# kyutai-labs/moshi

Measured on AMD Instinct MI355X. Metric: 12.5 Hz frames/s end-to-end Mimi+Moshi-7B, higher is better.
Workload: dtype bf16

## Files before the change

moshi_amd/csrc/lm_engine.hip:

```cpp
#include "lm_kernels.h"
#include "mmi_graph.h"

#include <math.h>
#include <stdio.h>
#include <map>

namespace {

struct GemmW {
    u32x4* wp = nullptr;
    int N = 0, K = 0, NT = 0, KSTEPS = 0, gate = 0;
    float* scale = nullptr;
    float* scb = nullptr;
    int wq = 0;
    int ksteps = 0;
    uint8_t* s4 = nullptr;
    float xinv = 1.f;
    size_t bytes = 0;
    int T = 32;
};

struct LayerW {
    GemmW in_proj, out_proj, ffn_in, ffn_out;
    uint16_t *n1 = nullptr, *n2 = nullptr;
// ... 2224 lines not shown
        mx = off[b] > mx ? off[b] : mx;
    }
    hipStream_t s = (hipStream_t)stream;
    MMI_HIP_CHECK(hipStreamSynchronize(s));
    MMI_HIP_CHECK(hipMemcpy(lm->offsets, off.data(), (size_t)G * sizeof(long), hipMemcpyHostToDevice));
    if (lm->offsets_m != lm->offsets) MMI_HIP_CHECK(hipMemcpy(lm->offsets_m, off.data(), (size_t)lm->batch * sizeof(long), hipMemcpyHostToDevice));
    lm->offset_cpu = mx;
    lm->depth_bound = mx;
    return MMI_OK;
}

#define MMI_DBG_HIP(call)                                                                                          \
    do {                                                                                                           \
        hipError_t e_ = (call);                                                                                    \
        if (e_ != hipSuccess) return done(mmi_fail(MMI_ERR_HIP, std::string(#call) + ": " + hipGetErrorString(e_))); \
    } while (0)
#define MMI_DBG_LAUNCHED()                                                                                         \
    do {                                                                                                           \
        hipError_t e_ = hipGetLastError();                                                                         \
        if (e_ != hipSuccess) return done(mmi_fail(MMI_ERR_HIP, std::string("kernel launch failed: ") + hipGetErrorString(e_))); \
    } while (0)

extern "C" int mmi_lm_debug_linear(mmi_lm* lm, const char* weight_name, const char* alpha_name, int32_t path, const void* x_bf16,
                                   int32_t rows, void* out_bf16, int8_t* codes, float* absmax, void* norm_out, mmi_stream stream) {
    MmiDeviceGuard dev_guard_(lm ? lm->device : -1);
    if (!lm || !weight_name || !x_bf16 || !out_bf16) return mmi_fail(MMI_ERR_INVALID, "null argument");
    if (rows <= 0 || rows > lm->max_batch) return mmi_fail(MMI_ERR_SHAPE, "mmi_lm_debug_linear: rows must be 1..max_batch");
    auto it = lm->linear_by_name.find(weight_name);
    if (it == lm->linear_by_name.end()) return mmi_fail(MMI_ERR_MISSING_WEIGHT, std::string("no packed linear named ") + weight_name);
    const GemmW g = it->second;
    const uint16_t* alpha = nullptr;
    const bool normed = path == MMI_DBG_NORM || path == MMI_DBG_NORM_FUSED;
    if (normed) {
        auto ia = alpha_name ? lm->vector_by_name.find(alpha_name) : lm->vector_by_name.end();
        if (ia == lm->vector_by_name.end()) return mmi_fail(MMI_ERR_MISSING_WEIGHT, "mmi_lm_debug_linear: the norm's alpha vector was not found");
        alpha = ia->second;
    }
    const bool a8 = act8_of(lm);
    if ((codes || absmax) && !(a8 && (path == MMI_DBG_PLAIN || path == MMI_DBG_SPLITK || path == MMI_DBG_NORM)))
        return mmi_fail(MMI_ERR_UNSUPPORTED, "mmi_lm_debug_linear: codes / absmax exist on the int8 x int8 paths that materialise the operand (plain, split-K, norm)");
    hipStream_t s = (hipStream_t)stream;
    const int T = g.T, mt = mmi_cdiv(rows, T), KS = mmi_kstep(T);
    if (mt > 2 && (path == MMI_DBG_FUSED || path == MMI_DBG_NORM_FUSED))
        return mmi_fail(MMI_ERR_UNSUPPORTED, "mmi_lm_debug_linear: the fused forms are not selected above 64 rows (k_gemm_rows + a norm launch)");
    const int K = g.K, N = g.N, kin = packed_ksteps_t(lm, T, K), kout = packed_ksteps_t(lm, T, N);
    const int nthK = [&] { int n = mmi_cdiv(K / 8, 64) * 64; return n > 1024 ? 1024 : n; }();
    MmiArena A;
    A.poison = lm->knobs.debug_poison;
    uint16_t *xp = nullptr, *yp = nullptr, *xres = nullptr, *zeros = nullptr, *outp = (uint16_t*)out_bf16;
    uint8_t* xq = nullptr;
    float *sx = nullptr, *partial = nullptr;
    const size_t xelems = (size_t)mt * kin * 512, oelems = (size_t)mt * kout * 512;
    bool ok = true;
    ok &= hipSuccess == A.alloc(&xp, xelems);
    ok &= hipSuccess == A.alloc(&yp, xelems);
    ok &= hipSuccess == A.alloc(&xq, (size_t)mt * (kin / 2 + 1) * 1024);
    ok &= hipSuccess == A.alloc(&sx, (size_t)mt * T);
    ok &= hipSuccess == A.alloc(&xres, oelems);
    ok &= hipSuccess == A.alloc(&zeros, (size_t)N + 8);
    ok &= hipSuccess == A.alloc(&partial, (size_t)4 * rows * N);
    auto done = [&](int rc) { hipStreamSynchronize(s); A.release(); return rc; };
    if (!ok) return done(mmi_fail(MMI_ERR_HIP, "out of device memory (mmi_lm_debug_linear)"));
    MMI_DBG_HIP(hipMemsetAsync(xp, 0, xelems * 2, s));
    MMI_DBG_HIP(hipMemsetAsync(yp, 0, xelems * 2, s));
    MMI_DBG_HIP(hipMemsetAsync(xq, 0, (size_t)mt * (kin / 2 + 1) * 1024, s));
    MMI_DBG_HIP(hipMemsetAsync(sx, 0, (size_t)mt * T * sizeof(float), s));
    MMI_DBG_HIP(hipMemsetAsync(xres, 0, oelems * 2, s));
    MMI_DBG_HIP(hipMemsetAsync(zeros, 0, ((size_t)N + 8) * 2, s));
    MMI_LAUNCH(k_pack_rows, mmi_cdiv(rows * K, 256), 256, 0, s, (const uint16_t*)x_bf16, rows, K, xp, T, kin);
    MMI_DBG_LAUNCHED();
    const uint16_t* operand = xp;
    const bool gated = g.gate != 0;
    GemmArgs a;
    memset(&a, 0, sizeof(a));
    a.out = outp; a.epi = gated ? MMI_EPI_GATE : MMI_EPI_STORE; a.B = rows; a.tok_rows = rows;
    a.out_mode = MMI_OUT_ROWMAJOR; a.out_ld = N; a.out_ksteps = kout;
    int rc = MMI_OK;
    if (path == MMI_DBG_NORM) {
        MMI_LAUNCH(k_resid_rmsnorm, rows, nthK, 0, s, xp, (const float*)nullptr, 0, rows, alpha, yp, K, T, kin, 1e-8f,
                   a8 ? xq : (uint8_t*)nullptr, a8 ? sx : (float*)nullptr, (const float*)nullptr, (const float*)nullptr);
        MMI_DBG_LAUNCHED();
        operand = yp;
        if (norm_out) MMI_LAUNCH(k_unpack_rows, mmi_cdiv(rows * K, 256), 256, 0, s, (const uint16_t*)yp, rows, K, (uint16_t*)norm_out, T, kin);
    } else if (a8 && (path == MMI_DBG_PLAIN || path == MMI_DBG_SPLITK)) {
        MMI_LAUNCH(k_quant_rows_i8, rows, nthK, 0, s, (const uint16_t*)xp, rows, K, T, kin, xq, sx);
        MMI_DBG_LAUNCHED();
    }
    if (path == MMI_DBG_PLAIN || path == MMI_DBG_NORM || path == MMI_DBG_SPLITK) {
        a.xp = reinterpret_cast<const u32x4*>(operand);
        if (a8) { a.xp = reinterpret_cast<const u32x4*>(xq); a.sx = sx; a.wq = 3; }
        Pending pd;
        if (path == MMI_DBG_SPLITK) {
            const GemmPlan p = plan_gemm(lm->knobs, g, true);
            if (gated || p.ksplit <= 1) return done(mmi_fail(MMI_ERR_UNSUPPORTED, "mmi_lm_debug_linear: the engine does not split this GEMM over K"));
            a.epi = MMI_EPI_PARTIAL; a.partial = partial; a.out = nullptr;
            pd.P = p.ksplit;
            if (a8) { pd.sx = sx; pd.scb = g.scb; }
        }
        rc = launch_gemm(lm, s, g, a, false);
        if (rc) return done(rc);
        if (path == MMI_DBG_SPLITK) {
            const int nthN = [&] { int n = mmi_cdiv(N / 8, 64) * 64; return n > 1024 ? 1024 : n; }();
            if (N > 8 * 1024 * MMI_NORM_MAXP) return done(mmi_fail(MMI_ERR_UNSUPPORTED, "row too long for the norm kernel"));
            uint16_t* ytmp = nullptr;
            if (A.alloc(&ytmp, oelems) != hipSuccess) return done(mmi_fail(MMI_ERR_HIP, "out of device memory"));
            MMI_LAUNCH(k_resid_rmsnorm, rows, nthN, 0, s, xres, (const float*)partial, pd.P, rows, (const uint16_t*)zeros, ytmp, N, T, kout, 1e-8f,
                       (uint8_t*)nullptr, (float*)nullptr, pd.sx, pd.scb);
            MMI_LAUNCH(k_unpack_rows, mmi_cdiv(rows * N, 256), 256, 0, s, (const uint16_t*)xres, rows, N, outp, T, kout);
            MMI_DBG_LAUNCHED();
        }
    } else if (path == MMI_DBG_FUSED) {
        const int kmax = q8_fused_kmax(g);
        if (!a8 || !kmax) return done(mmi_fail(MMI_ERR_UNSUPPORTED, "mmi_lm_debug_linear: k_gemm_q8 needs an int8 x int8 model and rows of <= 88 entries"));
        a.xp = reinterpret_cast<const u32x4*>(xp);
        a.wp = g.wp; a.N = g.N; a.KSTEPS = g.KSTEPS; a.NT = g.NT; a.wscale = g.scale; a.wscb = g.scb; a.gate_rows = gated ? g.N : 0;
        a.wq = 3; a.xinv = g.xinv;
        a.osplit = q8_fused_osplit(lm->knobs, g, a.epi, T);
        rc = launch_q8_fused(s, T, mt, kmax, g.NT * a.osplit, !lm->knobs.q8_tiles_serial, a);
        if (rc) return done(rc);
    } else if (path == MMI_DBG_NORM_FUSED) {
        const int wq = (a8 && g.wq == 1) ? 3 : g.wq;
        if (g.KSTEPS > norm_fused_max(wq)) return done(mmi_fail(MMI_ERR_UNSUPPORTED, "mmi_lm_debug_linear: the row is too long for the norm-fused GEMM"));
        a.xp = reinterpret_cast<const u32x4*>(xp);
        a.alpha = alpha; a.D = K; a.eps = 1e-8f;
        a.wp = g.wp; a.N = g.N; a.KSTEPS = g.KSTEPS; a.NT = g.NT; a.wscale = g.scale; a.wscb = g.scb; a.ws4 = g.s4; a.gate_rows = gated ? g.N : 0;
        a.wq = wq; a.xinv = g.xinv; a.osplit = 1;
        rc = launch_norm_fused(s, T, mt, wq, g.NT, !lm->knobs.q8_tiles_serial, a);
        if (rc) return done(rc);
    } else {
        return done(mmi_fail(MMI_ERR_INVALID, "mmi_lm_debug_linear: unknown path"));
    }
    if (codes) MMI_LAUNCH(k_unpack_q8, mmi_cdiv(rows * K, 256), 256, 0, s, (const uint8_t*)xq, rows, K, codes, T, kin);
    if (absmax) MMI_DBG_HIP(hipMemcpyAsync(absmax, sx, (size_t)rows * sizeof(float), hipMemcpyDeviceToDevice, s));
    MMI_DBG_LAUNCHED();
    (void)KS;
    if (hipStreamSynchronize(s) != hipSuccess) { A.release(); return mmi_fail(MMI_ERR_HIP, "mmi_lm_debug_linear: the launches failed"); }
    A.release();
    return MMI_OK;
}

extern "C" int64_t mmi_lm_stat(const mmi_lm* lm, int32_t which) {
    MmiDeviceGuard dev_guard_(lm ? lm->device : -1);
    if (!lm) return -1;
    if (which == 0) return (int64_t)lm->xlds_launches;
    if (which == 1) {
        int64_t m = 0;
        for (int v = 0; v < MmiProgram::NV; ++v)
            if (lm->prog.ready(v, false) || lm->prog.ready(v, true)) m |= 1ll << v;
        return m;
    }
    if (which == 2) return (int64_t)lm->depth_bound;
    if (which == 3) return (int64_t)lm->Td;
    if (which == 4) return (int64_t)lm->rows_launches;
    return -1;
}

extern "C" int mmi_lm_profile_begin(mmi_lm* lm) {
    MmiDeviceGuard dev_guard_(lm ? lm->device : -1);
    if (!lm) return mmi_fail(MMI_ERR_INVALID, "null handle");
    lm->profiling = true;
    lm->ev_used = 0;
    lm->site_ev_used = 0;
    lm->prog.tap = [lm](size_t i, bool begin, hipStream_t s) {
        if (!begin && i + 1 != lm->prog.ops.size()) return;
        if (lm->site_ev_used == lm->site_ev.size()) {
            mmi_lm::SiteEv e{0, nullptr};
            if (hipEventCreate(&e.ev) != hipSuccess) return;
            lm->site_ev.push_back(e);
        }
        lm->site_ev[lm->site_ev_used].op = begin ? i : (size_t)-1;
        hipEventRecord(lm->site_ev[lm->site_ev_used].ev, s);
        lm->site_ev_used += 1;
    };
    return MMI_OK;
}

extern "C" int64_t mmi_lm_profile_sites(mmi_lm* lm, char* buf, int64_t cap) {
    MmiDeviceGuard dev_guard_(lm ? lm->device : -1);
    if (!lm || !lm->profiling) return 0;
    if (lm->prof_stream) hipStreamSynchronize(lm->prof_stream);
    else hipDeviceSynchronize();
    std::vector<std::string> order;
    std::vector<double> tot;
    std::vector<long> cnt, bytes;
    for (size_t k = 0; k + 1 < lm->site_ev_used; ++k) {
        const auto& e = lm->site_ev[k];
        if (e.op == (size_t)-1) continue;
        float ms = 0.f;
        if (hipEventElapsedTime(&ms, e.ev, lm->site_ev[k + 1].ev) != hipSuccess) continue;
        const std::string& site = lm->prog.sites[e.op];
        size_t j = 0;
        while (j < order.size() && order[j] != site) ++j;
        if (j == order.size()) { order.push_back(site); tot.push_back(0.0); cnt.push_back(0); bytes.push_back(0); }
        tot[j] += ms; cnt[j] += 1;
        if (lm->prog.op_bytes[e.op] > bytes[j]) bytes[j] = lm->prog.op_bytes[e.op];
    }
    (void)hipGetLastError();
    std::string all;
    for (size_t j = 0; j < order.size(); ++j)
        all += order[j] + "\t" + std::to_string(cnt[j]) + "\t" + std::to_string(tot[j]) + "\t" + std::to_string(bytes[j]) + "\n";
    const int64_t need = (int64_t)all.size() + 1;
    if (buf && cap > 0) {
        const int64_t n = need <= cap ? need - 1 : cap - 1;
        memcpy(buf, all.data(), (size_t)n);
        buf[n] = 0;
    }
    return need;
}

extern "C" int mmi_lm_profile_end(mmi_lm* lm, double* mean_ms, int64_t* n_launches, int64_t* bytes_per_launch,
                                  const char** kernel_name) {
    MmiDeviceGuard dev_guard_(lm ? lm->device : -1);
    if (!lm) return mmi_fail(MMI_ERR_INVALID, "null handle");
    if (!lm->profiling) return mmi_fail(MMI_ERR_STATE, "profiling was not started");
    lm->profiling = false;
    lm->prog.tap = nullptr;
    if (lm->prof_stream || lm->ev_used) MMI_HIP_CHECK(hipStreamSynchronize(lm->prof_stream));
    double tot = 0.0;
    for (size_t i = 0; i < lm->ev_used; ++i) {
        float ms = 0.f;
        MMI_HIP_CHECK(hipEventElapsedTime(&ms, lm->ev_pool[i].a, lm->ev_pool[i].b));
        tot += ms;
    }
    if (mean_ms) *mean_ms = lm->ev_used ? tot / (double)lm->ev_used : 0.0;
    if (n_launches) *n_launches = (int64_t)lm->ev_used;
    if (bytes_per_launch) {
        const mmi_lm_cfg& c = lm->cfg;
        const int64_t wbytes = lm->q8 == 4 ? (int64_t)2 * c.ffn_hidden * c.dim / 2 + (int64_t)2 * c.ffn_hidden * c.dim / 16
                               : lm->q8 >= 1 ? (int64_t)2 * c.ffn_hidden * c.dim + (int64_t)2 * c.ffn_hidden * 4 : (int64_t)2 * c.ffn_hidden * c.dim * 2;
        *bytes_per_launch = wbytes + (int64_t)lm->batch * c.dim * 2 + (int64_t)lm->batch * c.ffn_hidden * 2;
    }
    if (kernel_name)
        *kernel_name = lm->act8      ? "k_gemm_xp<32, MT, 1, 8, 2, 3> (temporal FFN linear_in, int8 weights x int8 activations on v_mfma_i32_32x32x32_i8 + SiLU gate)"
                       : lm->q8 == 1 ? "k_gemm_xp<32, 1, 1, 8, 2, 1> (temporal FFN linear_in, int8 weights + SiLU gate)"
                       : lm->q8 == 4 ? "k_gemm_xp<32, MT, 1, 8, U, 4> (temporal FFN linear_in, MXFP4 weights widened to bf16 + SiLU gate)"
                       : lm->q8 == 2 ? "k_gemm_xp<32, 1, 1, 8, 2, 2> (temporal FFN linear_in, fp8 weights on the fp8 MFMA + SiLU gate)"
                       : lm->dominant_xlds ? (lm->batch > 32 ? "k_gemm_xlds<2, 32, 3, true, 0> (temporal FFN linear_in + SiLU gate)"
                                                             : "k_gemm_xlds<1, 64, 3, true, 0> (temporal FFN linear_in + SiLU gate)")
                                     : "k_gemm_xp<32, 1, 1, 8, 2> (temporal FFN linear_in + SiLU gate)";
    lm->ev_used = 0;
    return MMI_OK;
}
```

moshi_amd/csrc/lm_kernels.h:

```cpp
#pragma once
#include "mmi_common.h"
#include "mmi_fp4.h"

MMI_HD long mmi_xp_index(int T, int b, int k, int ksteps) {
    const int sh = T == 32 ? 4 : 5;
    const int mt = b / T, bl = b - mt * T;
    const int ks = k >> sh, kq = (k >> 3) & ((1 << (sh - 3)) - 1), e = k & 7;
    return ((((long)mt * ksteps + ks) * 64) + kq * T + bl) * 8 + e;
}
static inline int mmi_kstep(int T) { return T == 32 ? 16 : 32; }

__global__ void k_pack_w_bf16(const uint16_t* __restrict__ W, uint16_t* __restrict__ P, int N, int K, int TN, int NT,
                              int KSTEPS, int gate_hidden) {
    long idx = (long)blockIdx.x * blockDim.x + threadIdx.x;
    long total = (long)NT * KSTEPS * 512;
    if (idx >= total) return;
    int e = (int)(idx & 7);
    int lane = (int)((idx >> 3) & 63);
    long rest = idx >> 9;
    int ks = (int)(rest % KSTEPS);
    int nt = (int)(rest / KSTEPS);
    int i, kq, kstep;
    if (TN == 32) { i = lane & 31; kq = lane >> 5; kstep = 16; } else { i = lane & 15; kq = lane >> 4; kstep = 32; }
    int k = ks * kstep + 8 * kq + e;
// ... 1521 lines not shown
    float max_period;
    unsigned* done;
    int solo_rows;
};

#define MMI_ATTN_CHUNK 256
template <int DH, bool KV8 = false>
__global__ __launch_bounds__(256) void k_lm_attn_split(LmAttnArgs a) {
    constexpr int EPL = KV8 ? 16 : 8;
    constexpr int ES = KV8 ? 1 : 2;
    constexpr int LPR = DH / EPL;
    constexpr int RPW = 64 / LPR;
    constexpr int CH = MMI_ATTN_CHUNK;
    const int bh = blockIdx.x;
    const int b = bh / a.H;
    const int tid = threadIdx.x, wave = tid >> 6, lane = tid & 63;
    const long off = a.offsets[b];
    const long end_new = off + 1;
    const int end_index = (int)(off % a.cap);
    const int L = (int)(end_new < (long)a.cap ? end_new : (long)a.cap);
    MMI_SHARED float sc[CH];
    MMI_SHARED float wred[8];
    MMI_SHARED float ored[4 * DH];
    const int seg = lane % LPR, rsub = lane / LPR;
    float qv[EPL];
#pragma unroll
    for (int v = 0; v < EPL / 8; ++v) {
        u32x4 qq = *reinterpret_cast<const u32x4*>(a.qrot + (long)bh * DH + seg * EPL + v * 8);
#pragma unroll
        for (int q = 0; q < 4; ++q) {
            qv[v * 8 + 2 * q] = mmi_bf16_to_f32((uint16_t)(qq[q] & 0xffffu));
            qv[v * 8 + 2 * q + 1] = mmi_bf16_to_f32((uint16_t)(qq[q] >> 16));
        }
    }
    auto widen = [](const u32x4& r, float* f) {
        if constexpr (KV8) {
#pragma unroll
            for (int q = 0; q < 4; ++q) mmi_fp8x4_to_f32(r[q], f + 4 * q);
        } else {
#pragma unroll
            for (int q = 0; q < 4; ++q) {
                f[2 * q] = mmi_bf16_to_f32((uint16_t)(r[q] & 0xffffu));
                f[2 * q + 1] = mmi_bf16_to_f32((uint16_t)(r[q] >> 16));
            }
        }
    };
    const uint8_t* kbase = reinterpret_cast<const uint8_t*>(a.kc) + (long)bh * a.cap * DH * ES;
    const uint8_t* vbase = reinterpret_cast<const uint8_t*>(a.vc) + (long)bh * a.cap * DH * ES;
    const float scale = 1.0f / sqrtf((float)DH);
    constexpr int PER_WAVE = CH / 4;
    float m_run = -INFINITY, l_run = 0.f;
    float acc[EPL];
#pragma unroll
    for (int e = 0; e < EPL; ++e) acc[e] = 0.f;
    for (int c0 = (int)blockIdx.y * CH; c0 < L; c0 += (int)gridDim.y * CH) {
        constexpr int NIT = PER_WAVE / RPW;
        constexpr int NB = NIT < 8 ? NIT : 8;
#pragma unroll 1
        for (int h0 = 0; h0 < NIT; h0 += NB) {
            u32x4 kk[NB];
#pragma unroll
            for (int i = 0; i < NB; ++i) {
                const int slot = min(c0 + wave * PER_WAVE + (h0 + i) * RPW + rsub, L - 1);
                kk[i] = *reinterpret_cast<const u32x4*>(kbase + ((long)slot * DH + seg * EPL) * ES);
            }
#pragma unroll
            for (int i = 0; i < NB; ++i) {
                const int rl = wave * PER_WAVE + (h0 + i) * RPW + rsub;
                const int slot = c0 + rl;
                bool valid = slot < L;
                if (valid) {
                    int delta = slot - end_index;
                    long pos = delta <= 0 ? off + delta : off + delta - a.cap;
                    long dq = off - pos;
                    valid = pos >= 0 && dq >= 0 && dq < a.context;
                }
                float dot = 0.f;
                float kf[EPL];
                widen(kk[i], kf);
#pragma unroll
                for (int e = 0; e < EPL; ++e) dot += qv[e] * kf[e];
#pragma unroll
                for (int m = LPR / 2; m >= 1; m >>= 1) dot += mmi_shfl_xor(dot, m);
                if (seg == 0) sc[rl] = valid ? dot * scale : -INFINITY;
            }
        }
        __syncthreads();
        const float sv = sc[tid];
        float mx = sv;
#pragma unroll
        for (int m = 32; m >= 1; m >>= 1) mx = fmaxf(mx, mmi_shfl_xor(mx, m));
        if (lane == 0) wred[wave] = mx;
        __syncthreads();
        mx = fmaxf(fmaxf(wred[0], wred[1]), fmaxf(wred[2], wred[3]));
        const float m_new = fmaxf(m_run, mx);
        const float p = (m_new == -INFINITY) ? 0.f : expf(sv - m_new);
        float sum = p;
#pragma unroll
        for (int m = 32; m >= 1; m >>= 1) sum += mmi_shfl_xor(sum, m);
        if (lane == 0) wred[4 + wave] = sum;
        sc[tid] = p;
        __syncthreads();
        sum = (wred[4] + wred[5]) + (wred[6] + wred[7]);
        const float resc = (m_run == -INFINITY) ? 0.f : expf(m_run - m_new);
        l_run = l_run * resc + sum;
        m_run = m_new;
#pragma unroll
        for (int e = 0; e < EPL; ++e) acc[e] *= resc;
#pragma unroll 1
        for (int h0 = 0; h0 < NIT; h0 += NB) {
            u32x4 vv[NB];
#pragma unroll
            for (int i = 0; i < NB; ++i) {
                const int slot = min(c0 + wave * PER_WAVE + (h0 + i) * RPW + rsub, L - 1);
                vv[i] = *reinterpret_cast<const u32x4*>(vbase + ((long)slot * DH + seg * EPL) * ES);
            }
#pragma unroll
            for (int i = 0; i < NB; ++i) {
                const int rl = wave * PER_WAVE + (h0 + i) * RPW + rsub;
                const float pr = (c0 + rl < L) ? sc[rl] : 0.f;
                float vf[EPL];
                widen(vv[i], vf);
#pragma unroll
                for (int e = 0; e < EPL; ++e) acc[e] += pr * vf[e];
            }
        }
        __syncthreads();
    }
#pragma unroll
    for (int e = 0; e < EPL; ++e)
#pragma unroll
        for (int m = 32; m >= LPR; m >>= 1) acc[e] += mmi_shfl_xor(acc[e], m);
    if (rsub == 0) {
#pragma unroll
        for (int e = 0; e < EPL; ++e) ored[wave * DH + seg * EPL + e] = acc[e];
    }
    __syncthreads();
    if (tid < DH) {
        const float o = (ored[tid] + ored[DH + tid]) + (ored[2 * DH + tid] + ored[3 * DH + tid]);
        if (gridDim.y == 1) {
            a.out[mmi_xp_index(a.T, b, (bh % a.H) * DH + tid, a.out_ksteps)] = mmi_f32_to_bf16(o / l_run);
        } else {
            a.opart[((long)bh * gridDim.y + blockIdx.y) * DH + tid] = o;
        }
    }
    if (gridDim.y > 1 && tid == 0) {
        float* mlp = a.ml + ((long)bh * gridDim.y + blockIdx.y) * 2;
        mlp[0] = m_run;
        mlp[1] = l_run;
    }
}

template <int DH, bool KV8 = false>
__global__ __launch_bounds__(256, KV8 ? 2 : 4) void k_lm_attn_wave(LmAttnArgs a) {
    constexpr int EPL = KV8 ? 16 : 8;
    constexpr int ES = KV8 ? 1 : 2;
    constexpr int LPR = DH / EPL;
    constexpr int RPW = 64 / LPR;
    constexpr int NB = 4;
    const int bh = blockIdx.x;
    const int b = bh / a.H;
    const int tid = threadIdx.x, wave = tid >> 6, lane = tid & 63;
    const long off = a.offsets[b];
    const int end_index = (int)(off % a.cap);
    const long end_new = off + 1;
    const int L = (int)(end_new < (long)a.cap ? end_new : (long)a.cap);
    const int seg = lane % LPR, rsub = lane / LPR;
    float qv[EPL];
    u32x4 qp = {0u, 0u, 0u, 0u};
#pragma unroll
    for (int v = 0; v < EPL / 8; ++v) {
        u32x4 qq = *reinterpret_cast<const u32x4*>(a.qrot + (long)bh * DH + seg * EPL + v * 8);
        if (v == 0) qp = qq;
#pragma unroll
        for (int q = 0; q < 4; ++q) {
            qv[v * 8 + 2 * q] = mmi_bf16_to_f32((uint16_t)(qq[q] & 0xffffu));
            qv[v * 8 + 2 * q + 1] = mmi_bf16_to_f32((uint16_t)(qq[q] >> 16));
        }
    }
    auto widen = [](const u32x4& r, float* f) {
        if constexpr (KV8) {
#pragma unroll
            for (int q = 0; q < 4; ++q) mmi_fp8x4_to_f32(r[q], f + 4 * q);
        } else {
#pragma unroll
            for (int q = 0; q < 4; ++q) {
                f[2 * q] = mmi_bf16_to_f32((uint16_t)(r[q] & 0xffffu));
                f[2 * q + 1] = mmi_bf16_to_f32((uint16_t)(r[q] >> 16));
            }
        }
    };
    const uint8_t* kbase = reinterpret_cast<const uint8_t*>(a.kc) + (long)bh * a.cap * DH * ES;
    const uint8_t* vbase = reinterpret_cast<const uint8_t*>(a.vc) + (long)bh * a.cap * DH * ES;
    const unsigned loff = (unsigned)(seg * EPL * ES);
    const float scale = 1.0f / sqrtf((float)DH);
    u32x4 kA[NB], vA[NB], kB[NB], vB[NB];
    const bool early = gridDim.y == 1;
    if (early) {
#pragma unroll
        for (int i = 0; i < NB; ++i) {
            const int slot_ = min((wave + i * 4) * RPW + rsub, a.cap - 1);
            const unsigned o_ = (unsigned)slot_ * (unsigned)(DH * ES) + loff;
            kA[i] = *reinterpret_cast<const u32x4*>(kbase + o_);
            vA[i] = *reinterpret_cast<const u32x4*>(vbase + o_);
        }
    }
    const bool windowed = a.context < a.cap;
    const bool solo = (int)gridDim.y > 1 && L <= a.solo_rows;
    if (solo && blockIdx.y != 0) return;
    const int nsplit = solo ? 1 : (int)gridDim.y;
    const int total = nsplit * 4, wg = (solo ? 0 : (int)blockIdx.y * 4) + wave;
    const int ngroups = (L + RPW - 1) / RPW;
    const int nmine = wg < ngroups ? (ngroups - wg + total - 1) / total : 0;
    const int nrounds = (nmine + NB - 1) / NB;
    float m_run = -INFINITY, l_run = 0.f, acc[EPL];
#pragma unroll
    for (int e = 0; e < EPL; ++e) acc[e] = 0.f;
#define MMI_AW_LOAD(KK, VV, j0)                                                                  \
    _Pragma("unroll") for (int i = 0; i < NB; ++i) {                                            \
        const int slot_ = min((wg + ((j0) + i) * total) * RPW + rsub, L - 1);                   \
        const unsigned o_ = (unsigned)slot_ * (unsigned)(DH * ES) + loff;                       \
        KK[i] = *reinterpret_cast<const u32x4*>(kbase + o_);                                    \
        VV[i] = *reinterpret_cast<const u32x4*>(vbase + o_);                                    \
    }
#define MMI_AW_USE(KK, VV, j0)                                                                   \
    {                                                                                            \
        float s_[NB];                                                                            \
        float mx_ = -INFINITY;                                                                   \
        _Pragma("unroll") for (int i = 0; i < NB; ++i) {                                        \
            const int j_ = (j0) + i;                                                             \
            const int slot_ = (wg + j_ * total) * RPW + rsub;                                    \
            bool valid_ = j_ < nmine && slot_ < L;                                               \
            if (windowed && valid_) {    \
                const int delta_ = slot_ - end_index;                                            \
                const long pos_ = delta_ <= 0 ? off + delta_ : off + delta_ - a.cap;             \
                const long dq_ = off - pos_;                                                     \
                valid_ = pos_ >= 0 && dq_ >= 0 && dq_ < a.context;                               \
            }                                                                                    \
            float dot_ = 0.f;                                                                    \
            if constexpr (KV8) {                                                                 \
                float kf_[EPL];                                                                  \
                widen(KK[i], kf_);                                                               \
                _Pragma("unroll") for (int e = 0; e < EPL; ++e) dot_ = mmi_fma(qv[e], kf_[e], dot_); \
            } else {                     \
                _Pragma("unroll") for (int q = 0; q < 4; ++q) dot_ = mmi_dot2_bf16(KK[i][q], qp[q], dot_); \
            }                                                                                    \
            dot_ = mmi_group_sum<LPR>(dot_);                 \
            s_[i] = valid_ ? dot_ * scale : -INFINITY;                                           \
            mx_ = fmaxf(mx_, s_[i]);                                                             \
        }                                                                                        \
        const float m_new_ = fmaxf(m_run, mx_);                                                  \
        if (m_new_ != -INFINITY) {                                                               \
            const float resc_ = m_run == -INFINITY ? 0.f : expf(m_run - m_new_);                 \
            l_run *= resc_;                                                                      \
            _Pragma("unroll") for (int e = 0; e < EPL; ++e) acc[e] *= resc_;                    \
            _Pragma("unroll") for (int i = 0; i < NB; ++i) {                                    \
                const float p_ = expf(s_[i] - m_new_);         \
                l_run += p_;                                                                     \
                if constexpr (KV8) {                                                             \
                    float vf_[EPL];                                                              \
                    widen(VV[i], vf_);                                                           \
                    _Pragma("unroll") for (int e = 0; e < EPL; ++e) acc[e] = mmi_fma(p_, vf_[e], acc[e]); \
                } else {                 \
                    const f32x2 pp_ = {p_, p_};                                                  \
                    _Pragma("unroll") for (int q = 0; q < 4; ++q) {                             \
                        const f32x2 v2_ = {__builtin_bit_cast(float, VV[i][q] << 16), __builtin_bit_cast(float, VV[i][q] & 0xffff0000u)}; \
                        const f32x2 a2_ = mmi_pk_fma(pp_, v2_, f32x2{acc[2 * q], acc[2 * q + 1]}); \
                        acc[2 * q] = a2_[0];                                                     \
                        acc[2 * q + 1] = a2_[1];                                                 \
                    }                                                                            \
                }                                                                                \
            }                                                                                    \
            m_run = m_new_;                                                                      \
        }                                                                                        \
    }
    if (nrounds > 0) {
        if (!early) { MMI_AW_LOAD(kA, vA, 0) }
        for (int r = 0; r < nrounds; r += 2) {
            MMI_AW_LOAD(kB, vB, (r + 1) * NB)
            MMI_AW_USE(kA, vA, r * NB)
            MMI_AW_LOAD(kA, vA, (r + 2) * NB)
            MMI_AW_USE(kB, vB, (r + 1) * NB)
        }
    }
#undef MMI_AW_LOAD
#undef MMI_AW_USE
#pragma unroll
    for (int mk = LPR; mk < 64; mk <<= 1) {
        const float mo = mmi_shfl_xor(m_run, mk), lo = mmi_shfl_xor(l_run, mk);
        const float mn = fmaxf(m_run, mo);
        const float sa = m_run == -INFINITY ? 0.f : expf(m_run - mn), sb = mo == -INFINITY ? 0.f : expf(mo - mn);
        l_run = l_run * sa + lo * sb;
#pragma unroll
        for (int e = 0; e < EPL; ++e) acc[e] = acc[e] * sa + mmi_shfl_xor(acc[e], mk) * sb;
        m_run = mn;
    }
    MMI_SHARED float wm[4], wl[4];
    MMI_SHARED float wacc[4 * DH];
    if (rsub == 0) {
#pragma unroll
        for (int e = 0; e < EPL; ++e) wacc[wave * DH + seg * EPL + e] = acc[e];
        if (seg == 0) { wm[wave] = m_run; wl[wave] = l_run; }
    }
    __syncthreads();
    if (tid < DH) {
        const float M = fmaxf(fmaxf(wm[0], wm[1]), fmaxf(wm[2], wm[3]));
        float num = 0.f, den = 0.f;
#pragma unroll
        for (int w = 0; w < 4; ++w) {
            const float sw = wm[w] == -INFINITY ? 0.f : expf(wm[w] - M);
            num += sw * wacc[w * DH + tid];
            den += sw * wl[w];
        }
        if (nsplit == 1) {
            a.out[mmi_xp_index(a.T, b, (bh % a.H) * DH + tid, a.out_ksteps)] = mmi_f32_to_bf16(num / den);
        } else {
            a.opart[((long)bh * gridDim.y + blockIdx.y) * DH + tid] = num;
            if (tid == 0) {
                float* mlp = a.ml + ((long)bh * gridDim.y + blockIdx.y) * 2;
                mlp[0] = M;
                mlp[1] = den;
            }
        }
    }
    if (nsplit == 1 || a.done == nullptr) return;
    MMI_SHARED unsigned s_last;
    __syncthreads();
    if (tid == 0) {
        const unsigned seen = mmi_arrive_release(a.done + bh);
        s_last = seen == (unsigned)gridDim.y - 1u ? 1u : 0u;
        if (s_last) {
            mmi_store_relaxed_agent(a.done + bh, 0u);
            mmi_acquire_agent();
        }
    }
    __syncthreads();
    if (!s_last) return;
    if (tid < DH) {
        const int NSg = (int)gridDim.y;
        const float* ml = a.ml + (long)bh * NSg * 2;
        float M = -INFINITY;
        for (int c = 0; c < NSg; ++c) M = fmaxf(M, ml[2 * c]);
        float num = 0.f, den = 0.f;
        for (int c = 0; c < NSg; ++c) {
            const float m = ml[2 * c];
            if (m == -INFINITY) continue;
            const float w = expf(m - M);
            num += w * a.opart[((long)bh * NSg + c) * DH + tid];
            den += w * ml[2 * c + 1];
        }
        a.out[mmi_xp_index(a.T, b, (bh % a.H) * DH + tid, a.out_ksteps)] = mmi_f32_to_bf16(num / den);
    }
}

__global__ void k_lm_attn_combine(LmAttnArgs a) {
    const int bh = blockIdx.x;
    const int Dh = a.Dh;
    const float* ml = a.ml + (long)bh * a.NS * 2;
    float M = -INFINITY;
    for (int c = 0; c < a.NS; ++c) M = fmaxf(M, ml[2 * c]);
    for (int d = threadIdx.x; d < Dh; d += blockDim.x) {
        float num = 0.f, den = 0.f;
        for (int c = 0; c < a.NS; ++c) {
            float m = ml[2 * c];
            if (m == -INFINITY) continue;
            float w = expf(m - M);
            num += w * a.opart[((long)bh * a.NS + c) * Dh + d];
            den += w * ml[2 * c + 1];
        }
        a.out[mmi_xp_index(a.T, bh / a.H, (bh % a.H) * Dh + d, a.out_ksteps)] = mmi_f32_to_bf16(num / den);
    }
}

struct DepAttnArgs {
    const uint16_t* qkv;
    uint16_t* kc;
    uint16_t* vc;
    uint16_t* out;
    int B, H, Dh, steps, k;
    int T, out_ksteps;
};

template <int ROWS>
__global__ __launch_bounds__(64) void k_dep_attn(DepAttnArgs a) {
    const int b = blockIdx.x / a.H, h = blockIdx.x % a.H;
    const int lane = threadIdx.x, Dh = a.Dh, HD = a.H * Dh;
    const bool on = lane < Dh;
    const uint16_t* row = a.qkv + (long)b * 3 * HD;
    uint16_t* kcb = a.kc + ((long)b * a.H + h) * a.steps * Dh;
    uint16_t* vcb = a.vc + ((long)b * a.H + h) * a.steps * Dh;
    float q = 0.f;
    uint16_t kn = 0, vn = 0;
    if (on) {
        q = mmi_bf16_to_f32(row[h * Dh + lane]);
        kn = row[HD + h * Dh + lane];
        vn = row[2 * HD + h * Dh + lane];
        kcb[(long)a.k * Dh + lane] = kn;
        vcb[(long)a.k * Dh + lane] = vn;
    }
    const float scale = 1.0f / sqrtf((float)Dh);
    float kr[ROWS], vr[ROWS];
#pragma unroll
    for (int j = 0; j < ROWS; ++j) {
        const int jc = j < a.k ? j : (a.k > 0 ? a.k - 1 : 0);
        const int lc = on ? lane : 0;
        kr[j] = mmi_bf16_to_f32(kcb[(long)jc * Dh + lc]);
        vr[j] = mmi_bf16_to_f32(vcb[(long)jc * Dh + lc]);
    }
    float sc[ROWS];
    float mx = -INFINITY;
#pragma unroll
    for (int j = 0; j < ROWS; ++j) {
        if (j <= a.k) {
            float kv = 0.f;
            if (on) kv = (j == a.k) ? mmi_bf16_to_f32(kn) : kr[j];
            float d = q * kv;
#pragma unroll
            for (int m = 32; m >= 1; m >>= 1) d += mmi_shfl_xor(d, m);
            sc[j] = d * scale;
            mx = fmaxf(mx, sc[j]);
        }
    }
    float den = 0.f, o = 0.f;
#pragma unroll
    for (int j = 0; j < ROWS; ++j) {
        if (j <= a.k) {
            float p = expf(sc[j] - mx);
            den += p;
            float vv = 0.f;
            if (on) vv = (j == a.k) ? mmi_bf16_to_f32(vn) : vr[j];
            o += p * vv;
        }
    }
    if (on) a.out[mmi_xp_index(a.T, b, h * Dh + lane, a.out_ksteps)] = mmi_f32_to_bf16(o / den);
}
// ... 1070 lines not shown
```

moshi_amd/csrc/mmi_common.h:

```cpp
#pragma once
#include <mmi_device.h>
#include "../../include/moshi_mi.h"
#include "mmi_knobs.h"

#include <stdint.h>
#include <stdlib.h>
#include <string.h>
#include <string>
#include <vector>
#include <functional>

#define MMI_HD __host__ __device__ __forceinline__
MMI_HD uint16_t mmi_f32_to_bf16_bits(float f);

MMI_HD float mmi_bf16_to_f32(uint16_t h) { return __builtin_bit_cast(float, (uint32_t)h << 16); }
MMI_HD uint16_t mmi_f32_to_bf16_bits(float f) {
    uint32_t u = __builtin_bit_cast(uint32_t, f);
    if ((u & 0x7fffffffu) > 0x7f800000u) return (uint16_t)((u >> 16) | 0x0040u);
    u += 0x7fffu + ((u >> 16) & 1u);
    return (uint16_t)(u >> 16);
}
MMI_HD uint16_t mmi_f32_to_bf16(float f) { return mmi_cvt_bf16(f); }
MMI_HD uint32_t mmi_pack_bf16x2(float lo, float hi) { return mmi_cvt_pk_bf16(lo, hi); }
MMI_HD float mmi_round_bf16(float f) { return mmi_bf16_to_f32(mmi_f32_to_bf16(f)); }

static inline int mmi_cdiv(int a, int b) { return (a + b - 1) / b; }
static inline int64_t mmi_cdiv64(int64_t a, int64_t b) { return (a + b - 1) / b; }

void mmi_set_error(const std::string& msg);
int mmi_fail(int code, const std::string& msg);

#define MMI_HIP_CHECK(expr)                                                                          \
    do {                                                                                             \
        hipError_t e_ = (expr);                                                                      \
        if (e_ != hipSuccess)                                                                        \
            return mmi_fail(MMI_ERR_HIP, std::string(#expr) + ": " + hipGetErrorString(e_));         \
    } while (0)

#define MMI_CHECK_LAUNCH()                                                                           \
    do {                                                                                             \
        hipError_t e_ = hipGetLastError();                                                           \
        if (e_ != hipSuccess)                                                                        \
            return mmi_fail(MMI_ERR_HIP, std::string("kernel launch: ") + hipGetErrorString(e_));    \
    } while (0)

struct MmiDeviceGuard {
    int prev = -1;
    explicit MmiDeviceGuard(int dev) {
        int cur = -1;
        if (dev >= 0 && hipGetDevice(&cur) == hipSuccess && cur != dev && hipSetDevice(dev) == hipSuccess) prev = cur;
    }
    ~MmiDeviceGuard() { if (prev >= 0) hipSetDevice(prev); }
    MmiDeviceGuard(const MmiDeviceGuard&) = delete;
    MmiDeviceGuard& operator=(const MmiDeviceGuard&) = delete;
};

struct MmiWeights {
    const mmi_tensor_desc* descs;
    int n;
    const mmi_tensor_desc* find(const std::string& name) const {
        for (int i = 0; i < n; ++i)
            if (descs[i].name && name == descs[i].name) return &descs[i];
        return nullptr;
    }
};

struct MmiArena {
    std::vector<void*> ptrs;
    std::vector<size_t> sizes;
    size_t bytes = 0;
    char poison = 0;
    template <class T>
    hipError_t alloc(T** p, size_t count) {
        void* q = nullptr;
        size_t nb = count * sizeof(T);
        if (nb == 0) nb = sizeof(T);
        hipError_t e = hipMalloc(&q, nb);
        if (e != hipSuccess) return e;
        if (poison && (e = hipMemset(q, poison == '1' ? 0xFF : 0x00, nb)) != hipSuccess) { hipFree(q); return e; }
        ptrs.push_back(q);
        sizes.push_back(nb);
        bytes += nb;
        *p = (T*)q;
        return hipSuccess;
    }
    void release() {
        for (void* p : ptrs) hipFree(p);
        ptrs.clear();
        sizes.clear();
        bytes = 0;
    }
    hipError_t save(void* dst, hipStream_t s) const {
        size_t at = 0;
        for (size_t i = 0; i < ptrs.size(); ++i) {
            hipError_t e = hipMemcpyAsync((char*)dst + at, ptrs[i], sizes[i], hipMemcpyDeviceToDevice, s);
            if (e != hipSuccess) return e;
            at += sizes[i];
        }
        return hipSuccess;
    }
    hipError_t load(const void* src, hipStream_t s) {
        size_t at = 0;
        for (size_t i = 0; i < ptrs.size(); ++i) {
            hipError_t e = hipMemcpyAsync(ptrs[i], (const char*)src + at, sizes[i], hipMemcpyDeviceToDevice, s);
            if (e != hipSuccess) return e;
            at += sizes[i];
        }
        return hipSuccess;
    }
};
```

Before: 4454.

## Peel attention prefetch tail, zero invalid V rows, raise KV8 occupancy

```diff
diff --git a/moshi_amd/csrc/lm_engine.hip b/moshi_amd/csrc/lm_engine.hip
--- a/moshi_amd/csrc/lm_engine.hip
+++ b/moshi_amd/csrc/lm_engine.hip
@@ -2400,6 +2400,8 @@
     if (which == 2) return (int64_t)lm->depth_bound;
     if (which == 3) return (int64_t)lm->Td;
     if (which == 4) return (int64_t)lm->rows_launches;
+    if ((which == 5 || which == 6) && lm->streaming)
+        return (int64_t)lm->st.snapshot_offset(which == 5 ? (const void*)lm->kc : (const void*)lm->vc);
     return -1;
 }
 
diff --git a/moshi_amd/csrc/lm_kernels.h b/moshi_amd/csrc/lm_kernels.h
--- a/moshi_amd/csrc/lm_kernels.h
+++ b/moshi_amd/csrc/lm_kernels.h
@@ -1697,7 +1697,7 @@
 }
 
 template <int DH, bool KV8 = false>
-__global__ __launch_bounds__(256, KV8 ? 2 : 4) void k_lm_attn_wave(LmAttnArgs a) {
+__global__ __launch_bounds__(256, KV8 ? 3 : 4) void k_lm_attn_wave(LmAttnArgs a) {
     constexpr int EPL = KV8 ? 16 : 8;
     constexpr int ES = KV8 ? 1 : 2;
     constexpr int LPR = DH / EPL;
@@ -1771,6 +1771,7 @@
 #define MMI_AW_USE(KK, VV, j0)                                                                   \
     {                                                                                            \
         float s_[NB];                                                                            \
+        bool ok_[NB];                                                                            \
         float mx_ = -INFINITY;                                                                   \
         _Pragma("unroll") for (int i = 0; i < NB; ++i) {                                        \
             const int j_ = (j0) + i;                                                             \
@@ -1792,7 +1793,13 @@
             }                                                                                    \
             dot_ = mmi_group_sum<LPR>(dot_);                 \
             s_[i] = valid_ ? dot_ * scale : -INFINITY;                                           \
+            ok_[i] = valid_;                                                                     \
             mx_ = fmaxf(mx_, s_[i]);                                                             \
+        }                                                                                        \
+         \
+        if (windowed || (wg + ((j0) + NB - 1) * total) * RPW + RPW > L) {                        \
+            _Pragma("unroll") for (int i = 0; i < NB; ++i)                                      \
+                if (!ok_[i]) VV[i] = u32x4{0u, 0u, 0u, 0u};                                      \
         }                                                                                        \
         const float m_new_ = fmaxf(m_run, mx_);                                                  \
         if (m_new_ != -INFINITY) {                                                               \
@@ -1821,11 +1828,28 @@
     }
     if (nrounds > 0) {
         if (!early) { MMI_AW_LOAD(kA, vA, 0) }
-        for (int r = 0; r < nrounds; r += 2) {
-            MMI_AW_LOAD(kB, vB, (r + 1) * NB)
-            MMI_AW_USE(kA, vA, r * NB)
-            MMI_AW_LOAD(kA, vA, (r + 2) * NB)
-            MMI_AW_USE(kB, vB, (r + 1) * NB)
+        if constexpr (KV8) {
+            for (int r = 0; r < nrounds; r += 2) {
+                MMI_AW_LOAD(kB, vB, (r + 1) * NB)
+                MMI_AW_USE(kA, vA, r * NB)
+                MMI_AW_LOAD(kA, vA, (r + 2) * NB)
+                MMI_AW_USE(kB, vB, (r + 1) * NB)
+            }
+        } else {
+            int r = 0;
+            for (; r + 2 < nrounds; r += 2) {
+                MMI_AW_LOAD(kB, vB, (r + 1) * NB)
+                MMI_AW_USE(kA, vA, r * NB)
+                MMI_AW_LOAD(kA, vA, (r + 2) * NB)
+                MMI_AW_USE(kB, vB, (r + 1) * NB)
+            }
+            if (r + 1 < nrounds) {
+                MMI_AW_LOAD(kB, vB, (r + 1) * NB)
+                MMI_AW_USE(kA, vA, r * NB)
+                MMI_AW_USE(kB, vB, (r + 1) * NB)
+            } else {
+                MMI_AW_USE(kA, vA, r * NB)
+            }
         }
     }
 #undef MMI_AW_LOAD
diff --git a/moshi_amd/csrc/mmi_common.h b/moshi_amd/csrc/mmi_common.h
--- a/moshi_amd/csrc/mmi_common.h
+++ b/moshi_amd/csrc/mmi_common.h
@@ -90,6 +90,14 @@
         sizes.clear();
         bytes = 0;
     }
+    long snapshot_offset(const void* p) const {
+        size_t at = 0;
+        for (size_t i = 0; i < ptrs.size(); ++i) {
+            if (ptrs[i] == p) return (long)at;
+            at += sizes[i];
+        }
+        return -1;
+    }
     hipError_t save(void* dst, hipStream_t s) const {
         size_t at = 0;
         for (size_t i = 0; i < ptrs.size(); ++i) {
```

New measurement: 4452. About the same (-0.0%).
